# rafaelghiorzi/YOLO-MS

Hardware: AMD Instinct MI355X
Metric: images/sec (train+infer) YOLO-MS-S 640x640 bf16 at 1/2/4/8 MI355X; mAP parity (higher is better)
Workload: dtype bf16; 1 GPU; configs[2]: YOLO-MS-S (reference YOLOv8-'s' graph) 640x640 bf16 training, B=64/GPU, fwd+loss+bwd+SGD-nesterov step; global_batch=64, per_gpu_batch=64, img=640, parallelism=dp1, hip_graph=False

## Files before the change

yolo-ms_amd/csrc/stem.hip:

```cpp
#include <algorithm>
#include <cstdlib>

#include "conv_common.hpp"

namespace yms {

constexpr int ST_TH = 8, ST_TW = 32;
constexpr int ST_IH = 2 * ST_TH + 1;
constexpr int ST_IW = 2 * ST_TW + 4;
constexpr int ST_IN = 3 * ST_IH * ST_IW;

struct StemParams {
  const float* x;
  const float* w;
  char* y;
  int y_ld, y_off;
  const float* scale;
  const float* shift;
  int act;
  float* stats;
  int stats_ld;
  float* stats_cnt;
  int N, CI, H, W, CO, Ho, Wo, tiles_x, tiles_y;
  int vec4;
  int ysplit, tps;
};

template <typename T>
__device__ __forceinline__ uint32_t pack2(float a, float b) {
  const T ta = (T)a, tb = (T)b;
  return (uint32_t)__builtin_bit_cast(uint16_t, ta) | ((uint32_t)__builtin_bit_cast(uint16_t, tb) << 16);
}

template <typename T, int NT, bool STATS>
__global__ __launch_bounds__(256) void conv_stem_kernel(StemParams p) {
  constexpr int CP = NT * 32;
  constexpr int OP = CP * (int)sizeof(T) + 16;
  constexpr int OUT_B = 4 * 64 * OP;
  constexpr int IN_B = ST_IN * 4;
  constexpr int RED_B = 4 * 3 * CP * 4;
  __shared__ __attribute__((aligned(16))) char smem[IN_B + OUT_B + RED_B];
  float* xin = reinterpret_cast<float*>(smem);
  float* red = reinterpret_cast<float*>(smem + IN_B + OUT_B);

  const int per_col = p.tiles_x * p.ysplit;
  const int n = blockIdx.x / per_col, rem = blockIdx.x - n * per_col;
  const int tx = rem % p.tiles_x, ty0 = (rem / p.tiles_x) * p.tps, ty1 = min(p.tiles_y, ty0 + p.tps);
  const int ox0 = tx * ST_TW;
  const int tid = threadIdx.x, lane = tid & 63, wave = tid >> 6;
  const int lr = lane & 31, lh = lane >> 5;
  const float* xn = p.x + (long)n * p.CI * p.H * p.W;
  const int ix0 = 2 * ox0;

  constexpr int NV = 3 * ST_IH * 16, NVI = (NV + 255) / 256;
  f32x4 v[NVI];
  float hcol = 0.f;
  auto load_tile = [&](int ty) {
    const int iy0 = 2 * ty * ST_TH - 1;
#pragma unroll
    for (int j = 0; j < NVI; ++j) {
      const int it = tid + 256 * j;
      const int row = it >> 4, q = it & 15;
      const int ci = row / ST_IH, iy = iy0 + row - ci * ST_IH, ix = ix0 + 4 * q;
      v[j] = f32x4{0.f, 0.f, 0.f, 0.f};
      if (it < NV && ci < p.CI && iy >= 0 && iy < p.H) {
        const float* src = xn + ((long)ci * p.H + iy) * p.W + ix;
        if (p.vec4) {
          if (ix < p.W) v[j] = *reinterpret_cast<const f32x4*>(src);
        } else {
#pragma unroll
          for (int e = 0; e < 4; ++e) v[j][e] = ix + e < p.W ? src[e] : 0.f;
        }
      }
    }
    if (tid < 3 * ST_IH) {
      const int ci = tid / ST_IH, iy = iy0 + tid - ci * ST_IH;
      hcol = (ci < p.CI && iy >= 0 && iy < p.H && ix0 >= 1) ? xn[((long)ci * p.H + iy) * p.W + ix0 - 1] : 0.f;
    }
  };

  const int K = p.CI * 9;
  u32x4 bfr[NT][2];
#pragma unroll
  for (int b = 0; b < NT; ++b) {
    const int co = 32 * b + lr;
#pragma unroll
    for (int s = 0; s < 2; ++s) {
      float wv[8];
#pragma unroll
      for (int j = 0; j < 8; ++j) {
        const int k = 16 * s + 8 * lh + j;
        wv[j] = (co < p.CO && k < K) ? p.w[(long)co * K + k] : 0.0f;
      }
      bfr[b][s] = u32x4{pack2<T>(wv[0], wv[1]), pack2<T>(wv[2], wv[3]), pack2<T>(wv[4], wv[5]),
                        pack2<T>(wv[6], wv[7])};
    }
  }
  int koff[2][8];
#pragma unroll
  for (int s = 0; s < 2; ++s)
#pragma unroll
    for (int j = 0; j < 8; ++j) {
      const int k = 16 * s + 8 * lh + j;
      const int ci = k / 9, t = k - ci * 9, kh = t / 3, kw = t - kh * 3;
      koff[s][j] = k < K ? (ci * ST_IH + kh) * ST_IW + kw + 3 : -1;
    }
  float sc[NT], sh[NT];
#pragma unroll
  for (int b = 0; b < NT; ++b) {
    const int co = 32 * b + lr;
    sc[b] = (!STATS && co < p.CO && p.scale) ? p.scale[co] : 1.0f;
    sh[b] = (!STATS && co < p.CO && p.shift) ? p.shift[co] : 0.0f;
  }
  auto prow = [&](int i) { return (i & 3) + 8 * (i >> 2) + 4 * lh; };
  const int vx = min(ST_TW, p.Wo - ox0);
  const int cch = p.CO / 8;
  T* y = reinterpret_cast<T*>(p.y);
  char* ot = smem + IN_B + wave * 64 * OP;

  load_tile(ty0);
  for (int ty = ty0; ty < ty1; ++ty) {
    const int oy0 = ty * ST_TH;
#pragma unroll
    for (int j = 0; j < NVI; ++j) {
      const int it = tid + 256 * j;
      if (it < NV) *reinterpret_cast<f32x4*>(xin + (it >> 4) * ST_IW + 4 + 4 * (it & 15)) = v[j];
    }
    if (tid < 3 * ST_IH) xin[tid * ST_IW + 3] = hcol;
    __syncthreads();
    if (ty + 1 < ty1) load_tile(ty + 1);
    f32x16 acc[2][NT];
#pragma unroll
    for (int a = 0; a < 2; ++a) {
#pragma unroll
      for (int b = 0; b < NT; ++b)
#pragma unroll
        for (int i = 0; i < 16; ++i) acc[a][b][i] = 0.0f;
      const int base = 2 * (2 * wave + a) * ST_IW + 2 * lr;
#pragma unroll
      for (int s = 0; s < 2; ++s) {
        float av[8];
#pragma unroll
        for (int j = 0; j < 8; ++j) av[j] = koff[s][j] >= 0 ? xin[base + koff[s][j]] : 0.0f;
        const u32x4 af = u32x4{pack2<T>(av[0], av[1]), pack2<T>(av[2], av[3]), pack2<T>(av[4], av[5]),
                               pack2<T>(av[6], av[7])};
#pragma unroll
        for (int b = 0; b < NT; ++b) acc[a][b] = Mfma<T>::mma(af, bfr[b][s], acc[a][b]);
      }
    }
    bool rowok[2];
#pragma unroll
    for (int a = 0; a < 2; ++a) rowok[a] = oy0 + 2 * wave + a < p.Ho;
    if constexpr (STATS) {
#pragma unroll
      for (int b = 0; b < NT; ++b) {
        float s = 0.f, cntv = 0.f;
#pragma unroll
        for (int a = 0; a < 2; ++a)
#pragma unroll
          for (int i = 0; i < 16; ++i)
            if (rowok[a] && prow(i) < vx) { s += acc[a][b][i]; cntv += 1.f; }
        s += __shfl_xor(s, 32);
        cntv += __shfl_xor(cntv, 32);
        const float mu = cntv > 0.f ? s / cntv : 0.f;
        float q = 0.f;
#pragma unroll
        for (int a = 0; a < 2; ++a)
#pragma unroll
          for (int i = 0; i < 16; ++i)
            if (rowok[a] && prow(i) < vx) {
              const float d = acc[a][b][i] - mu;
              q += d * d;
            }
        q += __shfl_xor(q, 32);
        if (lh == 0) {
          red[(wave * 3 + 0) * CP + 32 * b + lr] = cntv;
          red[(wave * 3 + 1) * CP + 32 * b + lr] = s;
          red[(wave * 3 + 2) * CP + 32 * b + lr] = q;
        }
      }
    }
#pragma unroll
    for (int b = 0; b < NT; ++b) {
      const int co = 32 * b + lr;
#pragma unroll
      for (int a = 0; a < 2; ++a)
#pragma unroll
        for (int i = 0; i < 16; ++i) {
          float val = acc[a][b][i];
          if (!STATS) {
            val = val * sc[b] + sh[b];
            if (p.act == YMS_ACT_SILU) val = silu_f(val);
          }
          *reinterpret_cast<T*>(ot + (a * 32 + prow(i)) * OP + co * (int)sizeof(T)) = (T)val;
        }
    }
    __syncthreads();
    if constexpr (STATS) {
      const int tile = (n * p.tiles_y + ty) * p.tiles_x + tx;
      if (tid < p.CO) {
        float nt = 0.f, st = 0.f;
#pragma unroll
        for (int w = 0; w < 4; ++w) { nt += red[(w * 3 + 0) * CP + tid]; st += red[(w * 3 + 1) * CP + tid]; }
        const float mean = nt > 0.f ? st / nt : 0.f;
        float m2 = 0.f;
#pragma unroll
        for (int w = 0; w < 4; ++w) {
          const float nw = red[(w * 3 + 0) * CP + tid];
          if (nw > 0.f) {
            const float d = red[(w * 3 + 1) * CP + tid] / nw - mean;
            m2 += red[(w * 3 + 2) * CP + tid] + nw * d * d;
          }
        }
        float* so = p.stats + (long)tile * 2 * p.stats_ld;
        so[tid] = st;
        so[p.stats_ld + tid] = m2;
        if (tid == 0) p.stats_cnt[tile] = nt;
      }
    }
    for (int it = lane; it < 64 * cch; it += 64) {
      const int px = it / cch, ch = it - px * cch;
      const int a = px >> 5, ox = ox0 + (px & 31), oy = oy0 + 2 * wave + a;
      if (oy < p.Ho && ox < p.Wo) {
        const u32x4 val = *reinterpret_cast<const u32x4*>(ot + px * OP + ch * 16);
        *reinterpret_cast<u32x4*>(y + (((long)n * p.Ho + oy) * p.Wo + ox) * p.y_ld + p.y_off + 8 * ch) = val;
      }
    }
  }
}

template <typename T, int NT>
__global__ __launch_bounds__(256) void conv_stem_wgrad_kernel(StemParams p, const T* gy, int gy_ld, int gy_off,
                                                              const T* z, int z_ld, int z_off, const float* mi,
                                                              const float* coef, float* ws) {
  constexpr int CP = NT * 32;
  constexpr int DP = 256 + 8;
  constexpr int IN_B = ST_IN * 4;
  constexpr int DZ_B = CP * DP * (int)sizeof(T);
  constexpr int RED_B = 4 * CP * 32 * 4;
  constexpr int MAIN_B = (IN_B + DZ_B) > RED_B ? (IN_B + DZ_B) : RED_B;
  __shared__ __attribute__((aligned(16))) char smem[MAIN_B + 4 * CP * 4];
  float* xin = reinterpret_cast<float*>(smem);
  T* dzt = reinterpret_cast<T*>(smem + IN_B);
  float* red = reinterpret_cast<float*>(smem);
  float (*prm)[CP] = reinterpret_cast<float (*)[CP]>(smem + MAIN_B);

  const int per_col = p.tiles_x * p.ysplit;
  const int n = blockIdx.x / per_col, rem = blockIdx.x - n * per_col;
  const int tx = rem % p.tiles_x, ty0 = (rem / p.tiles_x) * p.tps, ty1 = min(p.tiles_y, ty0 + p.tps);
  const int ox0 = tx * ST_TW;
  const int tid = threadIdx.x, lane = tid & 63, wave = tid >> 6;
  const int lr = lane & 31, lh = lane >> 5;
  const float* xn = p.x + (long)n * p.CI * p.H * p.W;
  const int ix0 = 2 * ox0, K = p.CI * 9, cch = p.CO / 8;

  constexpr int NPAIR = 128 * CP / 8, NDZ = (NPAIR + 255) / 256;
  for (int c = tid; c < CP; c += 256) {
    float sc = 0.f, sh = 0.f, a0 = 0.f, bz = 0.f;
    if (c < p.CO) {
      sc = p.scale[c];
      sh = p.shift[c];
      const float mu = mi[c], is = mi[p.CO + c];
      bz = -sc * coef[p.CO + c] * is;
      a0 = -sc * coef[c] - bz * mu;
    }
    prm[0][c] = sc; prm[1][c] = sh; prm[2][c] = a0; prm[3][c] = bz;
  }
  f32x16 acc[NT];
#pragma unroll
  for (int b = 0; b < NT; ++b)
#pragma unroll
    for (int i = 0; i < 16; ++i) acc[b][i] = 0.0f;
  const int kk = lr;
  const int kci = kk / 9, kt = kk - kci * 9, kkh = kt / 3, kkw = kt - kkh * 3;
  const bool kok = kk < K;

  constexpr int NV = 3 * ST_IH * 16, NVI = (NV + 255) / 256;
  f32x4 xv[NVI];
  float hcol = 0.f;
  Raw8<T> graw[NDZ][2], zraw[NDZ][2];
  auto load_tile = [&](int ty) {
    const int oy0 = ty * ST_TH, iy0 = 2 * oy0 - 1;
#pragma unroll
    for (int j = 0; j < NVI; ++j) {
      const int it = tid + 256 * j;
      const int row = it >> 4, q = it & 15;
      const int ci = row / ST_IH, iy = iy0 + row - ci * ST_IH, ix = ix0 + 4 * q;
      xv[j] = f32x4{0.f, 0.f, 0.f, 0.f};
      if (it < NV && ci < p.CI && iy >= 0 && iy < p.H) {
        const float* src = xn + ((long)ci * p.H + iy) * p.W + ix;
        if (p.vec4) {
          if (ix < p.W) xv[j] = *reinterpret_cast<const f32x4*>(src);
        } else {
#pragma unroll
          for (int e = 0; e < 4; ++e) xv[j][e] = ix + e < p.W ? src[e] : 0.f;
        }
      }
    }
    if (tid < 3 * ST_IH) {
      const int ci = tid / ST_IH, iy = iy0 + tid - ci * ST_IH;
      hcol = (ci < p.CI && iy >= 0 && iy < p.H && ix0 >= 1) ? xn[((long)ci * p.H + iy) * p.W + ix0 - 1] : 0.f;
    }
#pragma unroll
    for (int j = 0; j < NDZ; ++j) {
      const int it = tid + 256 * j;
      const int pp = it / (CP / 8), g = it - pp * (CP / 8);
      const int oy = oy0 + (pp >> 4), c0 = 8 * g;
#pragma unroll
      for (int h = 0; h < 2; ++h) {
        const int ox = ox0 + 2 * (pp & 15) + h;
#pragma unroll
        for (int k = 0; k < (int)(sizeof(T) / 2); ++k) { graw[j][h].v[k] = u32x4{0u, 0u, 0u, 0u}; zraw[j][h].v[k] = graw[j][h].v[k]; }
        if (it < NPAIR && g < cch && oy < p.Ho && ox < p.Wo) {
          const long pix = ((long)n * p.Ho + oy) * p.Wo + ox;
          load_raw8(gy + pix * gy_ld + gy_off + c0, 8, graw[j][h]);
          load_raw8(z + pix * z_ld + z_off + c0, 8, zraw[j][h]);
        }
      }
    }
  };

  load_tile(ty0);
  for (int ty = ty0; ty < ty1; ++ty) {
    __syncthreads();
#pragma unroll
    for (int j = 0; j < NVI; ++j) {
      const int it = tid + 256 * j;
      if (it < NV) *reinterpret_cast<f32x4*>(xin + (it >> 4) * ST_IW + 4 + 4 * (it & 15)) = xv[j];
    }
    if (tid < 3 * ST_IH) xin[tid * ST_IW + 3] = hcol;
#pragma unroll
    for (int j = 0; j < NDZ; ++j) {
      const int it = tid + 256 * j;
      if (it < NPAIR) {
        const int pp = it / (CP / 8), g = it - pp * (CP / 8), c0 = 8 * g;
        const int oy = ty * ST_TH + (pp >> 4);
        float o[2][8];
#pragma unroll
        for (int h = 0; h < 2; ++h) {
          const bool valid = g < cch && oy < p.Ho && ox0 + 2 * (pp & 15) + h < p.Wo;
          float gv[8], zv[8];
          unpack8(graw[j][h], gv);
          unpack8(zraw[j][h], zv);
#pragma unroll
          for (int e = 0; e < 8; ++e) {
            const int c = c0 + e;
            const float sc = prm[0][c], sh = prm[1][c], a0 = prm[2][c], bz = prm[3][c];
            float da = gv[e];
            if (p.act == YMS_ACT_SILU) da *= dsilu_f(zv[e] * sc + sh);
            o[h][e] = valid ? sc * da + a0 + bz * zv[e] : 0.f;
          }
        }
#pragma unroll
        for (int e = 0; e < 8; ++e)
          *reinterpret_cast<uint32_t*>(dzt + (c0 + e) * DP + 2 * pp) = pack2<T>(o[0][e], o[1][e]);
      }
    }
    __syncthreads();
    if (ty + 1 < ty1) load_tile(ty + 1);
#pragma unroll
    for (int a = 0; a < 2; ++a) {
      const int prow = 2 * wave + a;
#pragma unroll
      for (int s2 = 0; s2 < 2; ++s2) {
        const int p0 = 16 * s2 + 8 * lh;
        float bv[8];
        const int base = (kci * ST_IH + 2 * prow + kkh) * ST_IW + kkw + 3 + 2 * p0;
#pragma unroll
        for (int j = 0; j < 8; ++j) bv[j] = kok ? xin[base + 2 * j] : 0.f;
        const u32x4 bf = u32x4{pack2<T>(bv[0], bv[1]), pack2<T>(bv[2], bv[3]), pack2<T>(bv[4], bv[5]),
                               pack2<T>(bv[6], bv[7])};
#pragma unroll
        for (int b = 0; b < NT; ++b) {
          const u32x4 af = *reinterpret_cast<const u32x4*>(dzt + (32 * b + lr) * DP + 64 * wave + 32 * a + p0);
          acc[b] = Mfma<T>::mma(af, bf, acc[b]);
        }
      }
    }
  }
  __syncthreads();
#pragma unroll
  for (int b = 0; b < NT; ++b)
#pragma unroll
    for (int i = 0; i < 16; ++i) {
      const int co = 32 * b + (i & 3) + 8 * (i >> 2) + 4 * lh;
      red[(wave * CP + co) * 32 + lr] = acc[b][i];
    }
  __syncthreads();
  for (int it = tid; it < p.CO * K; it += 256) {
    const int co = it / K, k = it - co * K;
    const float v = ((red[(0 * CP + co) * 32 + k] + red[(1 * CP + co) * 32 + k]) + red[(2 * CP + co) * 32 + k]) +
                    red[(3 * CP + co) * 32 + k];
    ws[(long)blockIdx.x * p.CO * K + it] = v;
  }
}

__global__ __launch_bounds__(1024) void stem_wgrad_reduce_kernel(const float* ws, int blocks, int items, float* dw,
                                                                 int accumulate) {
  __shared__ float red[16][64];
  const int lane = threadIdx.x & 63, w = threadIdx.x >> 6;
  const int j = blockIdx.x * 64 + lane;
  float s0 = 0.f, s1 = 0.f, s2 = 0.f, s3 = 0.f;
  if (j < items) {
    int b = w;
    for (; b + 48 < blocks; b += 64) {
      s0 += ws[(long)b * items + j];
      s1 += ws[(long)(b + 16) * items + j];
      s2 += ws[(long)(b + 32) * items + j];
      s3 += ws[(long)(b + 48) * items + j];
    }
    for (; b < blocks; b += 16) s0 += ws[(long)b * items + j];
  }
  red[w][lane] = (s0 + s1) + (s2 + s3);
  __syncthreads();
  for (int h = 8; h >= 1; h >>= 1) {
    if (w < h) red[w][lane] += red[w + h][lane];
    __syncthreads();
  }
  if (w == 0 && j < items) dw[j] = accumulate ? dw[j] + red[0][lane] : red[0][lane];
}

static bool stem_shape_ok(const yms_conv_shape* s) {
  return s && s->n > 0 && s->h > 0 && s->w > 0 && s->cin >= 1 && s->cin <= 3 && s->cout >= 8 && s->cout % 8 == 0 &&
         s->cout <= 96 && s->k == 3 && s->stride == 2 && s->pad == 1 && s->ho == (s->h - 1) / 2 + 1 &&
         s->wo == (s->w - 1) / 2 + 1 && (s->dtype == YMS_BF16 || s->dtype == YMS_F16);
}

static int stem_tiles(const yms_conv_shape* s, int& tx, int& ty) {
  tx = (s->wo + ST_TW - 1) / ST_TW;
  ty = (s->ho + ST_TH - 1) / ST_TH;
  return s->n * tx * ty;
}

static unsigned stem_strips(const yms_conv_shape* s, StemParams& p, long target) {
  const long cols = (long)s->n * p.tiles_x;
  const int want = (int)std::max(1l, std::min<long>(p.tiles_y, (target + cols - 1) / cols));
  p.tps = (p.tiles_y + want - 1) / want;
  p.ysplit = (p.tiles_y + p.tps - 1) / p.tps;
  return (unsigned)(cols * p.ysplit);
}

constexpr long STEM_WG_BLOCKS = 1024;

}

using namespace yms;

extern "C" {

int yms_conv_stem_supported(const yms_conv_shape* s) { return stem_shape_ok(s) ? 1 : 0; }

int yms_conv_stem_stats_rows(const yms_conv_shape* s) {
  if (!stem_shape_ok(s)) return 0;
  int tx, ty;
  return stem_tiles(s, tx, ty);
}

yms_status yms_conv_stem_fwd(const yms_conv_shape* s, const float* x, const float* w, void* y, int y_ld, int y_off,
                             const float* scale, const float* shift, int act, float* stats, int stats_ld,
                             void* stream) {
  if (!s || !x || !w || !y) return YMS_ERR_INVALID;
  if (!stem_shape_ok(s)) return YMS_ERR_UNSUPPORTED;
  if (y_ld % 8 || y_off % 8 || y_off + s->cout > y_ld) return YMS_ERR_INVALID;
  if (stats && stats_ld < s->cout) return YMS_ERR_INVALID;
  if ((long)s->n * s->cin * s->h * s->w >= (1l << 31)) return YMS_ERR_UNSUPPORTED;
  StemParams p{};
  p.x = x; p.w = w; p.y = (char*)y; p.y_ld = y_ld; p.y_off = y_off;
  p.scale = scale; p.shift = shift; p.act = act;
  p.stats = stats; p.stats_ld = stats_ld;
  p.N = s->n; p.CI = s->cin; p.H = s->h; p.W = s->w; p.CO = s->cout; p.Ho = s->ho; p.Wo = s->wo;
  const int tiles = stem_tiles(s, p.tiles_x, p.tiles_y);
  p.vec4 = (s->w % 4 == 0 && ((uintptr_t)x & 15) == 0) ? 1 : 0;
  if (stats) p.stats_cnt = stats + (long)tiles * 2 * stats_ld;
  const unsigned blocks = stem_strips(s, p, 1024);
  hipStream_t st = (hipStream_t)stream;
  const int nt = (s->cout + 31) / 32;
#define YMS_STEM(TT)                                                                                         \
  do {                                                                                                       \
    if (stats) {                                                                                             \
      if (nt == 1) hipLaunchKernelGGL((conv_stem_kernel<TT, 1, true>), dim3(blocks), dim3(256), 0, st, p);    \
      else if (nt == 2) hipLaunchKernelGGL((conv_stem_kernel<TT, 2, true>), dim3(blocks), dim3(256), 0, st, p); \
      else hipLaunchKernelGGL((conv_stem_kernel<TT, 3, true>), dim3(blocks), dim3(256), 0, st, p);            \
    } else {                                                                                                 \
      if (nt == 1) hipLaunchKernelGGL((conv_stem_kernel<TT, 1, false>), dim3(blocks), dim3(256), 0, st, p);   \
      else if (nt == 2) hipLaunchKernelGGL((conv_stem_kernel<TT, 2, false>), dim3(blocks), dim3(256), 0, st, p); \
      else hipLaunchKernelGGL((conv_stem_kernel<TT, 3, false>), dim3(blocks), dim3(256), 0, st, p);           \
    }                                                                                                        \
  } while (0)
  if (s->dtype == YMS_BF16) YMS_STEM(bf16);
  else YMS_STEM(f16);
#undef YMS_STEM
  return launch_status();
}

size_t yms_conv_stem_wgrad_ws_bytes(const yms_conv_shape* s) {
  if (!stem_shape_ok(s)) return 0;
  StemParams p{};
  stem_tiles(s, p.tiles_x, p.tiles_y);
  return (size_t)stem_strips(s, p, STEM_WG_BLOCKS) * s->cout * s->cin * 9 * sizeof(float);
}

yms_status yms_conv_stem_wgrad(const yms_conv_shape* s, const float* x, const void* gy, int gy_ld, int gy_off,
                               const void* z, int z_ld, int z_off, const float* scale, const float* shift,
                               const float* mean_invstd, const float* coef, int act, float* ws, size_t ws_bytes,
                               float* dw, int accumulate, void* stream) {
  if (!s || !x || !gy || !z || !scale || !shift || !mean_invstd || !coef || !ws || !dw) return YMS_ERR_INVALID;
  if (!stem_shape_ok(s)) return YMS_ERR_UNSUPPORTED;
  if (gy_ld % 8 || gy_off % 8 || gy_off + s->cout > gy_ld || z_ld % 8 || z_off % 8 || z_off + s->cout > z_ld)
    return YMS_ERR_INVALID;
  if (ws_bytes < yms_conv_stem_wgrad_ws_bytes(s)) return YMS_ERR_INVALID;
  if ((long)s->n * s->cin * s->h * s->w >= (1l << 31)) return YMS_ERR_UNSUPPORTED;
  StemParams p{};
  p.x = x; p.scale = scale; p.shift = shift; p.act = act;
  p.N = s->n; p.CI = s->cin; p.H = s->h; p.W = s->w; p.CO = s->cout; p.Ho = s->ho; p.Wo = s->wo;
  stem_tiles(s, p.tiles_x, p.tiles_y);
  p.vec4 = (s->w % 4 == 0 && ((uintptr_t)x & 15) == 0) ? 1 : 0;
  const unsigned blocks = stem_strips(s, p, STEM_WG_BLOCKS);
  hipStream_t st = (hipStream_t)stream;
  const int nt = (s->cout + 31) / 32;
#define YMS_STEM_WG(TT)                                                                                        \
  do {                                                                                                         \
    const TT* g_ = (const TT*)gy; const TT* z_ = (const TT*)z;                                                 \
    if (nt == 1) hipLaunchKernelGGL((conv_stem_wgrad_kernel<TT, 1>), dim3(blocks), dim3(256), 0, st, p, g_, gy_ld, \
                                    gy_off, z_, z_ld, z_off, mean_invstd, coef, ws);                          \
    else if (nt == 2) hipLaunchKernelGGL((conv_stem_wgrad_kernel<TT, 2>), dim3(blocks), dim3(256), 0, st, p, g_, \
                                         gy_ld, gy_off, z_, z_ld, z_off, mean_invstd, coef, ws);              \
    else hipLaunchKernelGGL((conv_stem_wgrad_kernel<TT, 3>), dim3(blocks), dim3(256), 0, st, p, g_, gy_ld,    \
                            gy_off, z_, z_ld, z_off, mean_invstd, coef, ws);                                  \
  } while (0)
  if (s->dtype == YMS_BF16) YMS_STEM_WG(bf16);
  else YMS_STEM_WG(f16);
#undef YMS_STEM_WG
  yms_status e = launch_status();
  if (e != YMS_OK) return e;
  const int items = s->cout * s->cin * 9;
  hipLaunchKernelGGL(stem_wgrad_reduce_kernel, dim3((items + 63) / 64), dim3(1024), 0, st, ws, (int)blocks, items, dw,
                     accumulate);
  return launch_status();
}

}
```

Before: 3927 images/sec.

## Use persistent flat tile walk for stem conv forward with buffer loads

Replaces the per-image strip grid of the stem conv forward kernel with a persistent grid sized to occupancy times CU count. Each block walks a contiguous range of flattened tiles and prefetches the next tile across image boundaries. Input loads now use raw buffer loads with out-of-bounds zeroing instead of branches, and the precomputed koff register array is replaced by compile-time tap offsets. A waves-per-EU hint is added for the single-tile variant. The aim is better load balance and fewer registers, at the cost of new env-var switches and a per-buffer size limit.

After: 3926 images/sec, median of 3. No clear change (-0.0%).

```diff
diff --git a/yolo-ms_amd/csrc/stem.hip b/yolo-ms_amd/csrc/stem.hip
--- a/yolo-ms_amd/csrc/stem.hip
+++ b/yolo-ms_amd/csrc/stem.hip
@@ -23,8 +23,52 @@
   float* stats_cnt;
   int N, CI, H, W, CO, Ho, Wo, tiles_x, tiles_y;
   int vec4;
+  int flat;
   int ysplit, tps;
 };
+
+__device__ __forceinline__ void stem_run(const StemParams& p, int& f0, int& f1) {
+  if (p.flat) {
+    const int tiles = p.N * p.tiles_x * p.tiles_y, g = (int)gridDim.x, b = (int)blockIdx.x;
+    const int q = tiles / g, r = tiles - q * g;
+    f0 = b * q + min(b, r);
+    f1 = f0 + q + (b < r ? 1 : 0);
+  } else {
+    const int per_col = p.tiles_x * p.ysplit;
+    const int n = blockIdx.x / per_col, rem = blockIdx.x - n * per_col;
+    const int tx = rem % p.tiles_x, ty0 = (rem / p.tiles_x) * p.tps, ty1 = min(p.tiles_y, ty0 + p.tps);
+    f0 = (n * p.tiles_x + tx) * p.tiles_y + ty0;
+    f1 = f0 + ty1 - ty0;
+  }
+}
+constexpr int stem_tap(int k) { return ((k / 9) * ST_IH + (k % 9) / 3) * ST_IW + (k % 9) % 3 + 3; }
+struct StemTile { int n, tx, ty; };
+__device__ __forceinline__ StemTile stem_tile(const StemParams& p, int f) {
+  const int per_img = p.tiles_x * p.tiles_y;
+  StemTile t;
+  t.n = f / per_img;
+  const int r = f - t.n * per_img;
+  t.tx = r / p.tiles_y;
+  t.ty = r - t.tx * p.tiles_y;
+  return t;
+}
+
+__device__ __forceinline__ f32x4 stem_ld16(__amdgpu_buffer_rsrc_t r, uint32_t voff) {
+#if defined(__HIP_DEVICE_COMPILE__)
+  return __builtin_bit_cast(f32x4, __builtin_amdgcn_raw_buffer_load_b128(r, voff, 0, 0));
+#else
+  (void)r; (void)voff;
+  return f32x4{0.f, 0.f, 0.f, 0.f};
+#endif
+}
+__device__ __forceinline__ float stem_ld4(__amdgpu_buffer_rsrc_t r, uint32_t voff) {
+#if defined(__HIP_DEVICE_COMPILE__)
+  return __builtin_bit_cast(float, __builtin_amdgcn_raw_buffer_load_b32(r, voff, 0, 0));
+#else
+  (void)r; (void)voff;
+  return 0.f;
+#endif
+}
 
 template <typename T>
 __device__ __forceinline__ uint32_t pack2(float a, float b) {
@@ -32,8 +76,10 @@
   return (uint32_t)__builtin_bit_cast(uint16_t, ta) | ((uint32_t)__builtin_bit_cast(uint16_t, tb) << 16);
 }
 
+constexpr int STEM_FWD_OCC = 3;
 template <typename T, int NT, bool STATS>
-__global__ __launch_bounds__(256) void conv_stem_kernel(StemParams p) {
+__global__ __launch_bounds__(256) __attribute__((amdgpu_waves_per_eu(NT == 1 ? STEM_FWD_OCC : 1, 8)))
+void conv_stem_kernel(StemParams p) {
   constexpr int CP = NT * 32;
   constexpr int OP = CP * (int)sizeof(T) + 16;
   constexpr int OUT_B = 4 * 64 * OP;
@@ -43,39 +89,38 @@
   float* xin = reinterpret_cast<float*>(smem);
   float* red = reinterpret_cast<float*>(smem + IN_B + OUT_B);
 
-  const int per_col = p.tiles_x * p.ysplit;
-  const int n = blockIdx.x / per_col, rem = blockIdx.x - n * per_col;
-  const int tx = rem % p.tiles_x, ty0 = (rem / p.tiles_x) * p.tps, ty1 = min(p.tiles_y, ty0 + p.tps);
-  const int ox0 = tx * ST_TW;
+  int f0, f1;
+  stem_run(p, f0, f1);
   const int tid = threadIdx.x, lane = tid & 63, wave = tid >> 6;
   const int lr = lane & 31, lh = lane >> 5;
-  const float* xn = p.x + (long)n * p.CI * p.H * p.W;
-  const int ix0 = 2 * ox0;
 
   constexpr int NV = 3 * ST_IH * 16, NVI = (NV + 255) / 256;
   f32x4 v[NVI];
-  float hcol = 0.f;
-  auto load_tile = [&](int ty) {
-    const int iy0 = 2 * ty * ST_TH - 1;
+  float hcol;
+  auto load_tile = [&](int f) {
+    const StemTile t = stem_tile(p, f);
+    const float* xn = p.x + (long)t.n * p.CI * p.H * p.W;
+    const int ix0 = 2 * t.tx * ST_TW, iy0 = 2 * t.ty * ST_TH - 1;
+    const __amdgpu_buffer_rsrc_t rs =
+        __builtin_amdgcn_make_buffer_rsrc((void*)xn, (short)0, p.CI * p.H * p.W * 4, NT_RSRC3);
 #pragma unroll
     for (int j = 0; j < NVI; ++j) {
       const int it = tid + 256 * j;
       const int row = it >> 4, q = it & 15;
       const int ci = row / ST_IH, iy = iy0 + row - ci * ST_IH, ix = ix0 + 4 * q;
-      v[j] = f32x4{0.f, 0.f, 0.f, 0.f};
-      if (it < NV && ci < p.CI && iy >= 0 && iy < p.H) {
-        const float* src = xn + ((long)ci * p.H + iy) * p.W + ix;
-        if (p.vec4) {
-          if (ix < p.W) v[j] = *reinterpret_cast<const f32x4*>(src);
-        } else {
-#pragma unroll
-          for (int e = 0; e < 4; ++e) v[j][e] = ix + e < p.W ? src[e] : 0.f;
-        }
-      }
-    }
-    if (tid < 3 * ST_IH) {
+      const bool rok = it < NV && ci < p.CI && iy >= 0 && iy < p.H;
+      const uint32_t off = (uint32_t)(((ci * p.H + iy) * p.W + ix) * 4);
+      if (p.vec4) {
+        v[j] = stem_ld16(rs, rok && ix < p.W ? off : NT_OOB);
+      } else {
+#pragma unroll
+        for (int e = 0; e < 4; ++e) v[j][e] = stem_ld4(rs, rok && ix + e < p.W ? off + 4 * e : NT_OOB);
+      }
+    }
+    {
       const int ci = tid / ST_IH, iy = iy0 + tid - ci * ST_IH;
-      hcol = (ci < p.CI && iy >= 0 && iy < p.H && ix0 >= 1) ? xn[((long)ci * p.H + iy) * p.W + ix0 - 1] : 0.f;
+      const bool ok = tid < 3 * ST_IH && ci < p.CI && iy >= 0 && iy < p.H && ix0 >= 1;
+      hcol = stem_ld4(rs, ok ? (uint32_t)(((ci * p.H + iy) * p.W + ix0 - 1) * 4) : NT_OOB);
     }
   };
 
@@ -96,15 +141,6 @@
                         pack2<T>(wv[6], wv[7])};
     }
   }
-  int koff[2][8];
-#pragma unroll
-  for (int s = 0; s < 2; ++s)
-#pragma unroll
-    for (int j = 0; j < 8; ++j) {
-      const int k = 16 * s + 8 * lh + j;
-      const int ci = k / 9, t = k - ci * 9, kh = t / 3, kw = t - kh * 3;
-      koff[s][j] = k < K ? (ci * ST_IH + kh) * ST_IW + kw + 3 : -1;
-    }
   float sc[NT], sh[NT];
 #pragma unroll
   for (int b = 0; b < NT; ++b) {
@@ -113,14 +149,15 @@
     sh[b] = (!STATS && co < p.CO && p.shift) ? p.shift[co] : 0.0f;
   }
   auto prow = [&](int i) { return (i & 3) + 8 * (i >> 2) + 4 * lh; };
-  const int vx = min(ST_TW, p.Wo - ox0);
   const int cch = p.CO / 8;
   T* y = reinterpret_cast<T*>(p.y);
   char* ot = smem + IN_B + wave * 64 * OP;
 
-  load_tile(ty0);
-  for (int ty = ty0; ty < ty1; ++ty) {
-    const int oy0 = ty * ST_TH;
+  auto tile_step = [&](int f) {
+    const StemTile tc = stem_tile(p, f);
+    const int n = tc.n, tx = tc.tx, ty = tc.ty;
+    const int ox0 = tx * ST_TW, oy0 = ty * ST_TH;
+    const int vx = min(ST_TW, p.Wo - ox0);
 #pragma unroll
     for (int j = 0; j < NVI; ++j) {
       const int it = tid + 256 * j;
@@ -128,7 +165,7 @@
     }
     if (tid < 3 * ST_IH) xin[tid * ST_IW + 3] = hcol;
     __syncthreads();
-    if (ty + 1 < ty1) load_tile(ty + 1);
+    if (f + 1 < f1) load_tile(f + 1);
     f32x16 acc[2][NT];
 #pragma unroll
     for (int a = 0; a < 2; ++a) {
@@ -141,7 +178,12 @@
       for (int s = 0; s < 2; ++s) {
         float av[8];
 #pragma unroll
-        for (int j = 0; j < 8; ++j) av[j] = koff[s][j] >= 0 ? xin[base + koff[s][j]] : 0.0f;
+        for (int j = 0; j < 8; ++j) {
+          const int k0 = 16 * s + j, k1 = k0 + 8;
+          const int o0 = stem_tap(k0), o1 = k1 < 27 ? stem_tap(k1) : o0;
+          const float a0 = xin[base + (lh ? o1 : o0)];
+          av[j] = (k1 >= 27 && lh) ? 0.0f : a0;
+        }
         const u32x4 af = u32x4{pack2<T>(av[0], av[1]), pack2<T>(av[2], av[3]), pack2<T>(av[4], av[5]),
                                pack2<T>(av[6], av[7])};
 #pragma unroll
@@ -226,7 +268,11 @@
         *reinterpret_cast<u32x4*>(y + (((long)n * p.Ho + oy) * p.Wo + ox) * p.y_ld + p.y_off + 8 * ch) = val;
       }
     }
-  }
+  };
+
+  if (f0 >= f1) return;
+  load_tile(f0);
+  for (int f = f0; f < f1; ++f) tile_step(f);
 }
 
 template <typename T, int NT>
@@ -442,6 +488,43 @@
 
 constexpr long STEM_WG_BLOCKS = 1024;
 
+static int stem_env(const char* name, int dflt) {
+  const char* e = getenv(name);
+  return e && *e ? atoi(e) : dflt;
+}
+static bool stem_flat() { return stem_env("YMS_STEM_WALK", 1) != 0; }
+static unsigned stem_flat_grid(long tiles, int occ) {
+  const int o = stem_env("YMS_STEM_OCC", 0);
+  if (o > 0) occ = std::min(o, 8);
+  return (unsigned)std::max(1l, std::min(tiles, (long)occ * conv_cu_count()));
+}
+
+template <typename T, int NT, bool STATS>
+static void launch_stem(const yms_conv_shape* s, StemParams& p, long tiles, hipStream_t st) {
+  auto k = conv_stem_kernel<T, NT, STATS>;
+  unsigned blocks;
+  p.flat = stem_flat() ? 1 : 0;
+  if (p.flat) {
+    static int occ = 0;
+    if (occ == 0) {
+      int o = 0;
+      if (hipOccupancyMaxActiveBlocksPerMultiprocessor(&o, k, 256, 0) != hipSuccess || o < 1) o = 1;
+      occ = std::min(o, STEM_FWD_OCC);
+    }
+    blocks = stem_flat_grid(tiles, occ);
+  } else {
+    blocks = stem_strips(s, p, 1024);
+  }
+  hipLaunchKernelGGL(k, dim3(blocks), dim3(256), 0, st, p);
+}
+template <typename T, bool STATS>
+static void launch_stem_nt(const yms_conv_shape* s, StemParams& p, long tiles, hipStream_t st) {
+  const int nt = (s->cout + 31) / 32;
+  if (nt == 1) launch_stem<T, 1, STATS>(s, p, tiles, st);
+  else if (nt == 2) launch_stem<T, 2, STATS>(s, p, tiles, st);
+  else launch_stem<T, 3, STATS>(s, p, tiles, st);
+}
+
 }
 
 using namespace yms;
@@ -464,6 +547,7 @@
   if (y_ld % 8 || y_off % 8 || y_off + s->cout > y_ld) return YMS_ERR_INVALID;
   if (stats && stats_ld < s->cout) return YMS_ERR_INVALID;
   if ((long)s->n * s->cin * s->h * s->w >= (1l << 31)) return YMS_ERR_UNSUPPORTED;
+  if ((long)s->cin * s->h * s->w * 4 >= (1l << 31)) return YMS_ERR_UNSUPPORTED;
   StemParams p{};
   p.x = x; p.w = w; p.y = (char*)y; p.y_ld = y_ld; p.y_off = y_off;
   p.scale = scale; p.shift = shift; p.act = act;
@@ -472,24 +556,14 @@
   const int tiles = stem_tiles(s, p.tiles_x, p.tiles_y);
   p.vec4 = (s->w % 4 == 0 && ((uintptr_t)x & 15) == 0) ? 1 : 0;
   if (stats) p.stats_cnt = stats + (long)tiles * 2 * stats_ld;
-  const unsigned blocks = stem_strips(s, p, 1024);
   hipStream_t st = (hipStream_t)stream;
-  const int nt = (s->cout + 31) / 32;
-#define YMS_STEM(TT)                                                                                         \
-  do {                                                                                                       \
-    if (stats) {                                                                                             \
-      if (nt == 1) hipLaunchKernelGGL((conv_stem_kernel<TT, 1, true>), dim3(blocks), dim3(256), 0, st, p);    \
-      else if (nt == 2) hipLaunchKernelGGL((conv_stem_kernel<TT, 2, true>), dim3(blocks), dim3(256), 0, st, p); \
-      else hipLaunchKernelGGL((conv_stem_kernel<TT, 3, true>), dim3(blocks), dim3(256), 0, st, p);            \
-    } else {                                                                                                 \
-      if (nt == 1) hipLaunchKernelGGL((conv_stem_kernel<TT, 1, false>), dim3(blocks), dim3(256), 0, st, p);   \
-      else if (nt == 2) hipLaunchKernelGGL((conv_stem_kernel<TT, 2, false>), dim3(blocks), dim3(256), 0, st, p); \
-      else hipLaunchKernelGGL((conv_stem_kernel<TT, 3, false>), dim3(blocks), dim3(256), 0, st, p);           \
-    }                                                                                                        \
-  } while (0)
-  if (s->dtype == YMS_BF16) YMS_STEM(bf16);
-  else YMS_STEM(f16);
-#undef YMS_STEM
+  if (s->dtype == YMS_BF16) {
+    if (stats) launch_stem_nt<bf16, true>(s, p, tiles, st);
+    else launch_stem_nt<bf16, false>(s, p, tiles, st);
+  } else {
+    if (stats) launch_stem_nt<f16, true>(s, p, tiles, st);
+    else launch_stem_nt<f16, false>(s, p, tiles, st);
+  }
   return launch_status();
 }
 
```
